# fani-lab/OpeNTF

Measured on AMD Instinct MI355X. Metric: teams/sec (train) bnn_emb d=128 on DBLP, higher is better.
Workload: dtype f32 (fp16x3 split products, f32 accumulate)

## Files before the change

opentf_amd/csrc/ntf_fused_dw.hip:

```cpp
#include "ntf_fused_common.h"

namespace ntf {

struct DwArgs {
    int B, M, Bpad;
    const float *__restrict__ dzT, *__restrict__ h, *__restrict__ hs, *__restrict__ mu, *__restrict__ rho;
    const float* wp;
    const uint32_t* sbits; int nCB; uint32_t so_k0, so_k1; int so_inj;
    float *__restrict__ g_mu, *__restrict__ g_rho, *__restrict__ g_b, *__restrict__ g_bp;
    float klw;
    float *__restrict__ w_mu, *__restrict__ w_rho, *__restrict__ m_mu, *__restrict__ v_mu, *__restrict__ m_rho, *__restrict__ v_rho;
    float lr_over_bc1, b1, b2, eps, bc2_sqrt;
    int wg_begin;
    int* rflag; int rmode;
    const uint32_t* sT;
    const uint32_t* sinT;
    const uint16_t* hb;
    float a_scale, unscale;
    int ksplit; float* part; int64_t slab; int part_row0;
    unsigned long long* stamps;
    int ntile, stagger;
    NormalSpec cur_eps; int lean;
    int produce; NormalSpec nx_eps; float* nx_wp; uint16_t *nx_pl_wp, *nx_pl_mu; float nx_pscale; double nx_klw; double* nx_kl; int* nx_rflag;
};

__device__ __forceinline__ float adam_update(float p, float g, float& m, float& v, float lr_over_bc1, float b1, float b2, float eps, float bc2_sqrt) {
    adam_step(p, g, m, v, lr_over_bc1, b1, b2, eps, __builtin_amdgcn_rcpf(bc2_sqrt));
    return p;
}

__device__ __forceinline__ uint32_t transpose32(uint32_t a, int il) {
    uint32_t m = 0x0000FFFFu;
#pragma unroll
    for (int j = 16; j != 0; j >>= 1) {
        const uint32_t pv = (uint32_t)__shfl_xor((int)a, j, 64);
        const bool lower = (il & j) == 0;
        const uint32_t lo = lower ? a : pv, hi = lower ? pv : a;
        const uint32_t t = ((lo >> j) ^ hi) & m;
        a ^= lower ? (t << j) : t;
        m ^= m << (j >> 1);
    }
    return a;
}

__device__ __forceinline__ void dw_produce_next(const DwArgs& p, int64_t idx0, const float (&mu4)[4], const float (&rho4)[4], float& kl, float& amax) {
    float z[4], ov[4];
#if defined(DWQ_ABL) && (DWQ_ABL & 2)
    z[0] = z[1] = z[2] = z[3] = 1.f;
#else
    normal4(p.nx_eps, idx0 >> 2, idx0, INT64_MAX, z);
#endif
#pragma unroll
    for (int j = 0; j < 4; ++j) {
        float ls;
        const float sigma = softplus_rho_fast(rho4[j], ls);
        ov[j] = sigma * z[j];
        kl += -ls + 0.5f * (sigma * sigma + mu4[j] * mu4[j]) - 0.5f;
    }
    if (!p.lean) *reinterpret_cast<float4*>(p.nx_wp + idx0) = make_float4(ov[0], ov[1], ov[2], ov[3]);
    const int64_t row = idx0 >> 7; const int j = (int)(idx0 & 127);
    amax = fmaxf(amax, fmaxf(fmaxf(fabsf(ov[0]), fabsf(ov[1])), fmaxf(fabsf(ov[2]), fabsf(ov[3]))));
    amax = fmaxf(amax, fmaxf(fmaxf(fabsf(mu4[0]), fabsf(mu4[1])), fmaxf(fabsf(mu4[2]), fabsf(mu4[3]))));
    planes_store_quad(p.nx_pl_wp, row, j, 128, ov[0], ov[1], ov[2], ov[3], p.nx_pscale);
    planes_store_quad(p.nx_pl_mu, row, j, 128, mu4[0], mu4[1], mu4[2], mu4[3], p.nx_pscale);
}
__device__ __forceinline__ void dw_produce_next_fnn(const DwArgs& p, int64_t idx0, const float (&mu4)[4], float& amax) {
    const int64_t row = idx0 >> 7; const int j = (int)(idx0 & 127);
    amax = fmaxf(amax, fmaxf(fmaxf(fabsf(mu4[0]), fabsf(mu4[1])), fmaxf(fabsf(mu4[2]), fabsf(mu4[3]))));
    planes_store_quad(p.nx_pl_mu, row, j, 128, mu4[0], mu4[1], mu4[2], mu4[3], p.nx_pscale);
}
template <bool BAYES = true>
__device__ __forceinline__ void dw_produce_finish(const DwArgs& p, float kl, float amax, double* red, int nwaves) {
    if (!(amax * p.nx_pscale <= 65504.f)) *p.nx_rflag = 1;
    if (!BAYES) return;
    const double s = wave_reduce_sum_d((double)kl);
    __syncthreads();
    if ((threadIdx.x & 63) == 0) red[threadIdx.x >> 6] = s;
    __syncthreads();
    if (threadIdx.x == 0) { double t = 0.0; for (int w = 0; w < nwaves; ++w) t += red[w]; atomicAdd(p.nx_kl, t * p.nx_klw); }
}

template <int H, bool BAYES, bool ADAM, int HG = H>
__device__ __forceinline__ void out_dw_f32_body(const DwArgs& p, char* smem, int jh = 0) {
    constexpr int NJT = H / 32;
    constexpr int KB = 32;
    constexpr int HROW = 4 * H;
    constexpr int TA = DW_TC * KB * 4;
    constexpr int TH = KB * HROW;
    constexpr int STAGE = TA + (BAYES ? 2 : 1) * TH;
    const int tid = threadIdx.x, lane = tid & 63, wave = tid >> 6, il = lane & 31, half = lane >> 5;
    if (range_guard_skip(p.rflag, p.rmode, false)) return;
    const int c0 = (p.wg_begin + blockIdx.x) * DW_TC;
    const int crow = wave * 32 + il;
    const int c = c0 + crow;
    const int nib = p.Bpad / KB;

    f32x16 acc1[NJT], acc2[NJT];
#pragma unroll
    for (int j = 0; j < NJT; ++j)
#pragma unroll
        for (int r = 0; r < 16; ++r) { acc1[j][r] = 0.f; acc2[j][r] = 0.f; }
    float sum1 = 0.f, sum2 = 0.f;

    const uint32_t smem_base = lds_addr(smem);
    const int wave_u = __builtin_amdgcn_readfirstlane(wave);
    auto stage = [&](int ib, int buf) {
        const uint32_t sb = smem_base + buf * STAGE;
#pragma unroll
        for (int n = 0; n < TA / 1024 / DW_WAVES; ++n) {
            const int inst = wave_u * (TA / 1024 / DW_WAVES) + n;
            const int row = inst * 8 + (lane >> 3), pch = lane & 7;
            const int q = pch ^ ((row >> 1) & 7);
            glds16(p.dzT + ((int64_t)(c0 >> 8) * nib + ib) * 8192 + row * 32 + 4 * q, sb + inst * 1024);
        }
        constexpr int HI = TH / 1024;
#pragma unroll
        for (int n = 0; n < (HI + DW_WAVES - 1) / DW_WAVES; ++n) {
            const int inst = wave_u * ((HI + DW_WAVES - 1) / DW_WAVES) + n;
            if (inst < HI) {
                int64_t goff = (int64_t)ib * KB * H + inst * 256 + lane * 4;
                if constexpr (HG != H) { const int f = inst * 256 + lane * 4; goff = (int64_t)(ib * KB + f / H) * HG + jh * H + f % H; }
                glds16(p.h + goff, sb + TA + inst * 1024);
                if (BAYES) glds16(p.hs + goff, sb + TA + TH + inst * 1024);
            }
        }
    };

    const uint32_t cb = (uint32_t)((c0 + wave * 32) >> 5);
    auto sign_col_word = [&](int ib) -> uint32_t {
        const int i = ib * KB + il;
        uint32_t w = 0u;
        if (p.so_inj) { if ((int)cb < p.nCB) w = p.sbits[(int64_t)i * p.nCB + cb]; }
        else w = sign_word(p.so_k0, p.so_k1, (uint32_t)i, cb);
        return transpose32(w, il);
    };
    uint32_t word_next = 0;
    if (BAYES) word_next = sign_col_word(0);
    stage(0, 0);
    asm volatile("s_waitcnt vmcnt(0)" ::: "memory");
    __syncthreads();
    for (int ib = 0; ib < nib; ++ib) {
        const int buf = ib & 1;
        const uint32_t word = word_next >> (4 * half);
        if (BAYES && ib + 1 < nib) word_next = sign_col_word(ib + 1);
        if (ib + 1 < nib) stage(ib + 1, buf ^ 1);
        const char* sA = smem + buf * STAGE;
        const char* sH = sA + TA;
#pragma unroll
        for (int t = 0; t < 4; ++t) {
            const int q = 2 * t + half;
            const float4 a = *reinterpret_cast<const float4*>(sA + crow * 128 + 16 * (q ^ ((crow >> 1) & 7)));
            const float av[4] = {a.x, a.y, a.z, a.w};
#pragma unroll
            for (int e4 = 0; e4 < 4; ++e4) {
                const int kk = 8 * t + e4;
                const float a1 = av[e4];
                sum1 += a1;
                float a2 = a1;
                if (BAYES) { a2 = __uint_as_float(__float_as_uint(a1) ^ ((word << (31 - kk)) & 0x80000000u)); sum2 += a2; }
                const char* hb = sH + (kk + 4 * half) * HROW + 4 * NJT * il;
                float bv[NJT], bsv[NJT];
                if (NJT == 4) {
                    const float4 b4 = *reinterpret_cast<const float4*>(hb); bv[0] = b4.x; bv[1] = b4.y; bv[NJT > 2 ? 2 : 0] = b4.z; bv[NJT > 3 ? 3 : 0] = b4.w;
                    if (BAYES) { const float4 s4 = *reinterpret_cast<const float4*>(hb + TH); bsv[0] = s4.x; bsv[1] = s4.y; bsv[NJT > 2 ? 2 : 0] = s4.z; bsv[NJT > 3 ? 3 : 0] = s4.w; }
                } else if (NJT == 2) {
                    const float2 b2 = *reinterpret_cast<const float2*>(hb); bv[0] = b2.x; bv[NJT > 1 ? 1 : 0] = b2.y;
                    if (BAYES) { const float2 s2 = *reinterpret_cast<const float2*>(hb + TH); bsv[0] = s2.x; bsv[NJT > 1 ? 1 : 0] = s2.y; }
                } else {
                    bv[0] = *reinterpret_cast<const float*>(hb);
                    if (BAYES) bsv[0] = *reinterpret_cast<const float*>(hb + TH);
                }
#pragma unroll
                for (int jt = 0; jt < NJT; ++jt) {
                    acc1[jt] = __builtin_amdgcn_mfma_f32_32x32x2f32(a1, bv[jt], acc1[jt], 0, 0, 0);
// ... 214 lines not shown
        else if (ADAM) ld_vec<NJT>(p.w_mu + idx0, v_mu);
        float a_m1[NJT], a_v1[NJT], a_m2[NJT], a_v2[NJT];
        if (ADAM) { ld_vec<NJT>(p.m_mu + idx0, a_m1); ld_vec<NJT>(p.v_mu + idx0, a_v1); if (BAYES) { ld_vec<NJT>(p.m_rho + idx0, a_m2); ld_vec<NJT>(p.v_rho + idx0, a_v2); } }
#pragma unroll
        for (int jt = 0; jt < NJT; ++jt) {
            float gm = acc1[jt][r] * p.unscale, gr = 0.f, pm = 0.f, rh = 0.f;
            if (BAYES) {
                rh = v_rho[jt];
                pm = v_mu[jt];
                const float w = v_wp[jt];
                const RhoTerms t = rho_terms_fast<true>(rh);
                gm += p.klw * pm;
                const float s2 = acc2[jt][r] * p.unscale;
                gr = (t.lo ? s2 * w : s2 * (w * t.isig) * t.sg) + p.klw * t.kl_a * t.kl_b;
            } else if (ADAM) pm = v_mu[jt];
            o_mu[jt] = gm; o_rho[jt] = gr;
            if (ADAM) {
                o_mu[jt] = adam_update(pm, gm, a_m1[jt], a_v1[jt], p.lr_over_bc1, p.b1, p.b2, p.eps, p.bc2_sqrt);
                if (BAYES) o_rho[jt] = adam_update(rh, gr, a_m2[jt], a_v2[jt], p.lr_over_bc1, p.b1, p.b2, p.eps, p.bc2_sqrt);
            }
        }
        if (!ADAM) { st_vec<NJT>(p.g_mu + idx0, o_mu); if (BAYES) st_vec<NJT>(p.g_rho + idx0, o_rho); }
        else {
            st_vec<NJT>(p.w_mu + idx0, o_mu); st_vec<NJT>(p.m_mu + idx0, a_m1); st_vec<NJT>(p.v_mu + idx0, a_v1);
            if (BAYES) { st_vec<NJT>(p.w_rho + idx0, o_rho); st_vec<NJT>(p.m_rho + idx0, a_m2); st_vec<NJT>(p.v_rho + idx0, a_v2); }
        }
    }
}


constexpr int SWT_IB = 16;
__global__ __launch_bounds__(256) void k_sign_words_T(const uint32_t* __restrict__ sbits, int so_inj, uint32_t k0, uint32_t k1, int B, int nCB, int ncb_all, int nib,
                                                      uint32_t* __restrict__ sT) {
    const int lane = threadIdx.x & 63, il = lane & 31, half = lane >> 5;
    const int cb = (blockIdx.x * 4 + (threadIdx.x >> 6)) * 2 + half;
    if (cb >= ncb_all) return;
    const int c = cb * 32 + il;
    uint32_t* dst = sT + (int64_t)(c >> 8) * nib * 256 + (c & 255);
    const int ib_end = min(nib, (int)(blockIdx.y + 1) * SWT_IB);
    for (int ib = blockIdx.y * SWT_IB; ib < ib_end; ++ib) {
        const int i = ib * 32 + il;
        uint32_t w = 0u;
        if (i < B) {
            if (so_inj) { if (cb < nCB) w = sbits[(int64_t)i * nCB + cb]; }
            else w = sign_word(k0, k1, (uint32_t)i, (uint32_t)cb);
        }
        dst[(int64_t)ib * 256] = transpose32(w, il);
    }
}

template <int N> struct DwOps { float rho[N], mu[N], m1[N], v1[N], m2[N], v2[N]; };
template <bool BAYES, bool ADAM, int N>
__device__ __forceinline__ void dw_ops_load(const DwArgs& p, int64_t idx0, DwOps<N>& o) {
    if (BAYES) { ld_vec<N>((ADAM ? p.w_rho : p.rho) + idx0, o.rho); ld_vec<N>((ADAM ? p.w_mu : p.mu) + idx0, o.mu); }
    else if (ADAM) ld_vec<N>(p.w_mu + idx0, o.mu);
    if (ADAM) { ld_vec<N>(p.m_mu + idx0, o.m1); ld_vec<N>(p.v_mu + idx0, o.v1); if (BAYES) { ld_vec<N>(p.m_rho + idx0, o.m2); ld_vec<N>(p.v_rho + idx0, o.v2); } }
}
template <bool BAYES, bool ADAM, int N>
__device__ __forceinline__ void dw_finish_ops(const DwArgs& p, int64_t idx0, const float (&s1)[N], const float (&s2)[N], DwOps<N>& o, float& nx_kl, float& nx_amax) {
    static_assert(N == 4, "one Philox quad per call");
    float o_mu[N], o_rho[N], z[4] = {0.f, 0.f, 0.f, 0.f};
#if defined(DWQ_ABL) && (DWQ_ABL & 1)
    z[0] = z[1] = z[2] = z[3] = 1.f;
#else
    if (BAYES) normal4(p.cur_eps, idx0 >> 2, idx0, INT64_MAX, z);
#endif
#pragma unroll
    for (int jt = 0; jt < N; ++jt) {
        float gm = s1[jt], gr = 0.f, pm = 0.f, rh = 0.f;
        if (BAYES) {
            rh = o.rho[jt];
            pm = o.mu[jt];
            const RhoTerms t = rho_terms_fast<true>(rh);
            gm += p.klw * pm;
            gr = s2[jt] * z[jt] * t.sg + p.klw * t.kl_a * t.kl_b;
        } else if (ADAM) pm = o.mu[jt];
        o_mu[jt] = gm; o_rho[jt] = gr;
        if (ADAM) {
            o_mu[jt] = adam_update(pm, gm, o.m1[jt], o.v1[jt], p.lr_over_bc1, p.b1, p.b2, p.eps, p.bc2_sqrt);
            if (BAYES) o_rho[jt] = adam_update(rh, gr, o.m2[jt], o.v2[jt], p.lr_over_bc1, p.b1, p.b2, p.eps, p.bc2_sqrt);
        }
    }
    if (!ADAM) { st_vec<N>(p.g_mu + idx0, o_mu); if (BAYES) st_vec<N>(p.g_rho + idx0, o_rho); }
    else {
        st_vec<N>(p.w_mu + idx0, o_mu); st_vec<N>(p.m_mu + idx0, o.m1); st_vec<N>(p.v_mu + idx0, o.v1);
        if (BAYES) { st_vec<N>(p.w_rho + idx0, o_rho); st_vec<N>(p.m_rho + idx0, o.m2); st_vec<N>(p.v_rho + idx0, o.v2); }
        if constexpr (N == 4) { if (p.produce) { if constexpr (BAYES) dw_produce_next(p, idx0, o_mu, o_rho, nx_kl, nx_amax); else dw_produce_next_fnn(p, idx0, o_mu, nx_amax); } }
    }
}
template <bool BAYES, bool ADAM, int N>
__device__ __forceinline__ void dw_finish_vec(const DwArgs& p, int64_t idx0, const float (&s1)[N], const float (&s2)[N], float& nx_kl, float& nx_amax) {
    DwOps<N> o;
    dw_ops_load<BAYES, ADAM, N>(p, idx0, o);
    dw_finish_ops<BAYES, ADAM, N>(p, idx0, s1, s2, o, nx_kl, nx_amax);
}

template <bool BAYES, bool ADAM>
__global__ __launch_bounds__(256) void k_out_dw_finish(DwArgs p) {
    if (p.rflag && *p.rflag) return;
    const int64_t q = (int64_t)blockIdx.x * 256 + threadIdx.x, il0 = q * 4, idx0 = il0 + (int64_t)p.part_row0 * 128;
    const int64_t Mp = p.slab / 128;
    if (q < Mp && q + p.part_row0 < p.M) {
        const float* pb = p.part + (int64_t)p.ksplit * 2 * p.slab;
        float b1 = 0.f, b2 = 0.f;
        for (int s = 0; s < p.ksplit; ++s) { b1 += pb[(int64_t)(s * 2) * Mp + q]; if (BAYES) b2 += pb[(int64_t)(s * 2 + 1) * Mp + q]; }
        p.g_b[q + p.part_row0] = b1; if (BAYES) p.g_bp[q + p.part_row0] = b2;
    }
    float nx_kl = 0.f, nx_amax = 0.f;
    const bool produce = ADAM && p.produce;
    const bool live = il0 < p.slab && idx0 < (int64_t)p.M * 128;
    if (!live && !produce) return;
    float s1[4] = {0.f, 0.f, 0.f, 0.f}, s2[4] = {0.f, 0.f, 0.f, 0.f};
    if (live) {
    for (int s = 0; s < p.ksplit; ++s) {
        float t[4];
        ld_vec<4>(p.part + (int64_t)(s * 2) * p.slab + il0, t);
#pragma unroll
        for (int k = 0; k < 4; ++k) s1[k] += t[k];
        if (BAYES) {
            ld_vec<4>(p.part + (int64_t)(s * 2 + 1) * p.slab + il0, t);
#pragma unroll
            for (int k = 0; k < 4; ++k) s2[k] += t[k];
        }
    }
    dw_finish_vec<BAYES, ADAM, 4>(p, idx0, s1, s2, nx_kl, nx_amax);
    }
    if (produce) { __shared__ double red[4]; dw_produce_finish<BAYES>(p, nx_kl, nx_amax, red, 4); }
}

__host__ __device__ __forceinline__ int sin_word_bit(int r) { const int g = r >> 3, q = (r & 7) >> 1, o = r & 1; return 16 * o + 4 * g + 3 - q; }
__global__ void k_sin_words_T(const uint32_t* __restrict__ sinbits, int Bpad, uint32_t* __restrict__ sinT) {
    const int t = blockIdx.x * blockDim.x + threadIdx.x;
    if (t >= (Bpad >> 5) * 128) return;
    const int ib = t >> 7, j = t & 127;
    uint32_t w = 0u;
    for (int r = 0; r < 32; ++r) w |= ((sinbits[(int64_t)(ib * 32 + r) * 4 + (j >> 5)] >> (j & 31)) & 1u) << sin_word_bit(r);
    sinT[t] = w;
}

#ifndef DW_EPI_PD
#define DW_EPI_PD 1
#endif
#ifndef DWQ_PRIO
#define DWQ_PRIO 2
#endif
#ifndef DWQ_BRING
#define DWQ_BRING 2
#endif
#ifndef DWQ_PPG
#define DWQ_PPG 3
#endif
constexpr int QW = 4;
constexpr int QTC = 32 * QW;
template <bool BAYES, bool ADAM, bool STAMP = false, bool SPLIT = false>
__global__ __launch_bounds__(64 * QW, 2) void k_out_dw_q(DwArgs p) {
    extern __shared__ __attribute__((aligned(16))) char smem[];
    constexpr int H = 128, NJT = 4;
    constexpr int TA = QTC * 32 * 4;
    constexpr int PLANE = H * 64;
    constexpr int TB = 2 * PLANE;
    constexpr int SRC_TB = (BAYES ? 2 : 1) * TB;
    constexpr int TW = BAYES ? 1024 : 0;
    constexpr int STAGE = TA + TB + TW;
    typedef _Float16 h2_t __attribute__((ext_vector_type(2)));
    const int tid = threadIdx.x, lane = tid & 63, wave = tid >> 6, il = lane & 31, half = lane >> 5;
    if (p.rmode == 1 && __builtin_nontemporal_load(p.rflag) != 0) return;
    const int ntile_s = SPLIT ? (int)gridDim.x / p.ksplit : 0;
    const int ksi = SPLIT ? (int)blockIdx.x / ntile_s : 0;
    const int c0 = (p.wg_begin + (SPLIT ? (int)blockIdx.x % ntile_s : (int)blockIdx.x)) * QTC;
    const int crow = wave * 32 + il, c = c0 + crow;
    const int nib = p.Bpad / 32;
    const int ib0 = SPLIT ? (int)((int64_t)ksi * nib / p.ksplit) : 0, ib1 = SPLIT ? (int)((int64_t)(ksi + 1) * nib / p.ksplit) : nib;
    const uint32_t smem_base = lds_addr(smem);
    const int wave_u = __builtin_amdgcn_readfirstlane(wave);
    const char* hb = reinterpret_cast<const char*>(p.hb);
    unsigned long long st_t[4] = {0, 0, 0, 0};
    if (STAMP) st_t[0] = __builtin_amdgcn_s_memrealtime();
    uint32_t lds_base = 0u;
    if (STAMP || (p.stagger > 0 && (int)blockIdx.x < p.ntile)) asm volatile("s_getreg_b32 %0, hwreg(HW_REG_LDS_ALLOC, 0, 8)" : "=s"(lds_base));
    if (p.stagger > 0 && (int)blockIdx.x < p.ntile) {
        if (lds_base != 0u) {
            const uint64_t t0 = __builtin_amdgcn_s_memrealtime();
            while (__builtin_amdgcn_s_memrealtime() - t0 < (uint64_t)p.stagger) __builtin_amdgcn_s_sleep(64);
        }
    }

    const h2_t ones = {(_Float16)1.0f, (_Float16)1.0f};
    constexpr int NA = TA / 1024 / QW, NB = TB / 1024 / QW;
    const float* dz_tile = p.dzT + (int64_t)(c0 >> 8) * nib * 8192 + ((c0 & 255) << 5);
    const uint32_t* sw_src = BAYES ? (half == 0 ? p.sT + (int64_t)(c0 >> 8) * nib * 256 + (c0 & 255) + il * 4 : p.sinT + il * 4) : nullptr;
    const int sw_step = half == 0 ? 256 : 128;
    auto stage_piece = [&](int ib, int buf, int n) {
        const uint32_t sb = smem_base + buf * STAGE;
        if (n < NA) {
            const int inst = wave_u * NA + n;
            const int row = inst * 8 + (lane >> 3), pch = lane & 7;
            const int q = pch ^ ((row >> 1) & 7);
            glds16(dz_tile + (int64_t)ib * 8192 + row * 32 + 4 * q, sb + inst * 1024);
        } else {
            const char* src = hb + (size_t)ib * SRC_TB;
            const int inst = wave_u * NB + (n - NA);
            const int pos = inst * 1024 + lane * 16;
            const int j = (pos % PLANE) >> 6, cd = (pos >> 4) & 3;
            glds16(src + (pos & ~63) + 16 * (cd ^ ((j >> 2) & 3)), sb + TA + inst * 1024);
            if (BAYES && n == NA + NB - 1) glds16(sw_src + (int64_t)ib * sw_step, sb + TA + TB);
        }
    };
    float nx_kl = 0.f, nx_amax = 0.f;
    unsigned long long st_c[3] = {0, 0, 0}, c_prev = 0;
    auto cyc = [&]() -> unsigned long long {
        unsigned long long t;
        __builtin_amdgcn_sched_barrier(0);
        asm volatile("s_memtime %0\n\ts_waitcnt lgkmcnt(0)" : "=s"(t) :: "memory");
        __builtin_amdgcn_sched_barrier(0);
        return t;
    };
#pragma unroll
    for (int n = 0; n < NA + NB; ++n) stage_piece(ib0, 0, n);
    f32x16 acc1[NJT], acc2[NJT];
#pragma unroll
    for (int j = 0; j < NJT; ++j)
#pragma unroll
        for (int r = 0; r < 16; ++r) { acc1[j][r] = 0.f; acc2[j][r] = 0.f; }
    float sum1 = 0.f, sum2 = 0.f;
    const int shl0 = 12 - 4 * half, shl1 = 4 - 4 * half;
    asm volatile("s_waitcnt vmcnt(0)" ::: "memory");
    __syncthreads();
    auto k_block = [&](int ib, auto more_c) {
        constexpr bool MORE = decltype(more_c)::value;
        const int buf = (ib - ib0) & 1;
        const char* sA = smem + buf * STAGE;
        const char* sB = sA + TA;
        uint32_t word = 0u;
        u32x4 iw = {0u, 0u, 0u, 0u};
        if (BAYES) { word = *reinterpret_cast<const uint32_t*>(sA + TA + TB + crow * 4); iw = *reinterpret_cast<const u32x4*>(sA + TA + TB + 512 + il * 16); }
        constexpr int NG = 2 * NJT;
        const char* bbase = sB + il * 64;
        const int swz = (il >> 2) & 3;
        auto load_b = [&](int g, u32x4 (&dst)[2]) {
            const int ks = g / NJT, jt = g % NJT;
            const char* bp = bbase + jt * 2048 + 16 * ((2 * ks + half) ^ swz);
#pragma unroll
            for (int q = 0; q < 2; ++q) dst[q] = *reinterpret_cast<const u32x4*>(bp + q * PLANE);
        };
        u32x4 a[2][2], as[2][2];
        auto prep_a = [&](int ks) {
            const int ch = 4 * ks + 2 * half, sw = (crow >> 1) & 7;
            const u32x4 lo = *reinterpret_cast<const u32x4*>(sA + crow * 128 + 16 * (ch ^ sw));
            const u32x4 hi = *reinterpret_cast<const u32x4*>(sA + crow * 128 + 16 * ((ch + 1) ^ sw));
            const uint32_t x[8] = {lo[0], lo[1], lo[2], lo[3], hi[0], hi[1], hi[2], hi[3]};
            const uint32_t w8 = word >> (ks * 16 + half * 8);
#pragma unroll
            for (int q = 0; q < 4; ++q) {
                const uint32_t p1 = __builtin_amdgcn_perm(x[2 * q + 1], x[2 * q], 0x05040100u), p2 = __builtin_amdgcn_perm(x[2 * q + 1], x[2 * q], 0x07060302u);
                a[ks][0][q] = p1; a[ks][1][q] = p2;
                sum1 = __builtin_amdgcn_fdot2(__builtin_bit_cast(h2_t, p1), ones, sum1, false);
                sum1 = __builtin_amdgcn_fdot2(__builtin_bit_cast(h2_t, p2), ones, sum1, false);
                if (BAYES) {
                    const uint32_t m = ((w8 << (15 - 2 * q)) & 0x8000u) | ((w8 << (30 - 2 * q)) & 0x80000000u);
                    const uint32_t s1 = p1 ^ m, s2 = p2 ^ m;
                    as[ks][0][q] = s1; as[ks][1][q] = s2;
                    sum2 = __builtin_amdgcn_fdot2(__builtin_bit_cast(h2_t, s1), ones, sum2, false);
                    sum2 = __builtin_amdgcn_fdot2(__builtin_bit_cast(h2_t, s2), ones, sum2, false);
                }
            }
        };
        constexpr int BR = DWQ_BRING;
        u32x4 bq[BR][2], bs[2];
#pragma unroll
        for (int g = 0; g < BR - 1; ++g) load_b(g, bq[g]);
        prep_a(0);
        int piece = 0;
        auto dma = [&]() {
            if (MORE) {
#pragma unroll
                for (int q = 0; q < DWQ_PPG; ++q) { if (piece < NA + NB) stage_piece(ib + 1, buf ^ 1, piece); ++piece; }
            }
        };
#pragma unroll
        for (int g = 0; g < NG; ++g) {
            if (g + BR - 1 < NG) load_b(g + BR - 1, bq[(g + BR - 1) % BR]);
            asm volatile("" ::: "memory");
            const int ks = g / NJT, jt = g % NJT;
            acc1[jt] = mfma3h(a[ks], bq[g % BR], acc1[jt]);
            dma();
            if (BAYES) {
                const uint32_t v = iw[jt] << (ks ? shl1 : shl0);
#pragma unroll
                for (int q = 0; q < 4; ++q) {
                    const uint32_t m = (v << q) & 0x80008000u;
                    bs[0][q] = bq[g % BR][0][q] ^ m; bs[1][q] = bq[g % BR][1][q] ^ m;
                }
                acc2[jt] = mfma3h(as[ks], bs, acc2[jt]);
                dma();
            }
            if (g == 0) prep_a(1);
        }
        if (STAMP) { st_c[0] += cyc() - c_prev; c_prev = cyc(); }
        asm volatile("s_waitcnt vmcnt(0)" ::: "memory");
        if (STAMP) { st_c[1] += cyc() - c_prev; c_prev = cyc(); }
        __syncthreads();
        if (STAMP) { st_c[2] += cyc() - c_prev; c_prev = cyc(); }
    };
    if (STAMP) { st_t[1] = __builtin_amdgcn_s_memrealtime(); c_prev = cyc(); }
    if (DWQ_PRIO) __builtin_amdgcn_s_setprio(DWQ_PRIO);
    for (int ib = ib0; ib < ib1 - 1; ++ib) k_block(ib, std::true_type{});
    k_block(ib1 - 1, std::false_type{});
    if (DWQ_PRIO) __builtin_amdgcn_s_setprio(0);
    if (STAMP) st_t[2] = __builtin_amdgcn_s_memrealtime();
    sum1 += __shfl_xor(sum1, 32, 64);
    sum2 += __shfl_xor(sum2, 32, 64);
    const float inv_a = 1.f / p.a_scale;
    if constexpr (SPLIT) {
        if (half == 0 && c < p.M) {
            float* pb = p.part + (int64_t)p.ksplit * 2 * p.slab; const int64_t Mp = p.slab / 128; const int cl = c - p.part_row0;
            pb[(int64_t)(ksi * 2) * Mp + cl] = sum1 * inv_a; if (BAYES) pb[(int64_t)(ksi * 2 + 1) * Mp + cl] = sum2 * inv_a;
        }
#pragma unroll
        for (int r = 0; r < 16; ++r) {
            const int cr = c0 + wave * 32 + rowmap(r, half);
            if (cr >= p.M) continue;
            const int64_t il0 = (int64_t)(cr - p.part_row0) * H + NJT * il;
            float s1[NJT], s2[NJT];
#pragma unroll
            for (int jt = 0; jt < NJT; ++jt) { s1[jt] = acc1[jt][r] * p.unscale; s2[jt] = acc2[jt][r] * p.unscale; }
            st_vec<NJT>(p.part + (int64_t)(ksi * 2) * p.slab + il0, s1);
            if (BAYES) st_vec<NJT>(p.part + (int64_t)(ksi * 2 + 1) * p.slab + il0, s2);
        }
        return;
    }
    if (half == 0 && c < p.M) { p.g_b[c] = sum1 * inv_a; if (BAYES) p.g_bp[c] = sum2 * inv_a; }

    constexpr int PD = DW_EPI_PD;
    DwOps<NJT> ops[PD + 1];
    auto row_idx = [&](int r, int64_t& idx0) -> bool {
        const int cr = c0 + wave * 32 + rowmap(r, half);
        idx0 = (int64_t)cr * H + NJT * il;
        return cr < p.M;
    };
    static_for<0, PD>([&](auto rc) { constexpr int r = decltype(rc)::value; int64_t idx0; if (row_idx(r, idx0)) dw_ops_load<BAYES, ADAM, NJT>(p, idx0, ops[r % (PD + 1)]); });
    static_for<0, 16>([&](auto rc) {
        constexpr int r = decltype(rc)::value;
        if constexpr (r + PD < 16) { int64_t idn; if (row_idx(r + PD, idn)) dw_ops_load<BAYES, ADAM, NJT>(p, idn, ops[(r + PD) % (PD + 1)]); }
        int64_t idx0;
        if (row_idx(r, idx0)) {
            float s1[NJT], s2[NJT];
#pragma unroll
            for (int jt = 0; jt < NJT; ++jt) { s1[jt] = acc1[jt][r] * p.unscale; s2[jt] = acc2[jt][r] * p.unscale; }
            dw_finish_ops<BAYES, ADAM, NJT>(p, idx0, s1, s2, ops[r % (PD + 1)], nx_kl, nx_amax);
        }
    });
    if (STAMP && p.stamps && lane == 0) {
        asm volatile("s_waitcnt vmcnt(0)" ::: "memory");
        st_t[3] = __builtin_amdgcn_s_memrealtime();
        uint32_t hw_id, xcc;
        asm volatile("s_getreg_b32 %0, hwreg(HW_REG_HW_ID)" : "=s"(hw_id));
        asm volatile("s_getreg_b32 %0, hwreg(HW_REG_XCC_ID)" : "=s"(xcc));
        unsigned long long* o = p.stamps + ((int64_t)blockIdx.x * QW + wave) * 10;
        o[0] = st_t[0]; o[1] = st_t[1]; o[2] = st_t[2]; o[3] = st_t[3]; o[4] = ((unsigned long long)xcc << 32) | hw_id; o[5] = lds_base;
        o[6] = st_c[0]; o[7] = st_c[1]; o[8] = st_c[2]; o[9] = 0;
    }
    if (ADAM && p.produce) dw_produce_finish<BAYES>(p, nx_kl, nx_amax, reinterpret_cast<double*>(smem + 2 * STAGE), QW);
}

void launch_fused_out_dw(hipStream_t st, const FusedDw& f) {
    const Geom g = geom(f.B, f.M);
    const WsLayout w = ws_layout(f.B, f.H, f.M);
    char* ws = static_cast<char*>(f.ws);
    DwArgs a;
    a.B = f.B; a.M = f.M; a.Bpad = g.Bpad; a.dzT = f.dzT; a.h = reinterpret_cast<const float*>(ws + w.hz); a.hs = reinterpret_cast<const float*>(ws + w.hs);
    a.mu = f.mu; a.rho = f.rho; a.wp = f.wp; a.sbits = reinterpret_cast<const uint32_t*>(ws + w.sbits); a.nCB = g.nCB;
    a.so_k0 = f.s_out.k0; a.so_k1 = f.s_out.k1; a.so_inj = f.s_out_inj;
    a.g_mu = f.g_mu; a.g_rho = f.g_rho; a.g_b = f.g_b; a.g_bp = f.g_bp; a.klw = f.klw;
    a.w_mu = f.w_mu; a.w_rho = f.w_rho; a.m_mu = f.m_mu; a.v_mu = f.v_mu; a.m_rho = f.m_rho; a.v_rho = f.v_rho;
    a.lr_over_bc1 = f.lr_over_bc1; a.b1 = f.b1; a.b2 = f.b2; a.eps = f.eps; a.bc2_sqrt = f.bc2_sqrt;
    const int total = (f.M + DW_TC - 1) / DW_TC;
    const int grid = f.wg_count > 0 ? std::min(f.wg_count, total - f.wg_begin) : total;
    a.wg_begin = f.wg_count > 0 ? f.wg_begin : 0;
    if (grid <= 0) return;
    a.hb = reinterpret_cast<const uint16_t*>(ws + w.hb);
    a.rflag = f.rflag; a.rmode = 0;
    a.produce = (f.produce && f.adam && f.H == 128) ? 1 : 0;
    a.cur_eps = f.cur_eps; a.lean = (a.produce && f.lean) ? 1 : 0;
    a.nx_eps = f.nx_eps; a.nx_wp = f.nx_wp; a.nx_pl_wp = f.nx_pl_wp; a.nx_pl_mu = f.nx_pl_mu; a.nx_pscale = f.nx_pscale; a.nx_klw = f.nx_klw; a.nx_kl = f.nx_kl; a.nx_rflag = f.nx_rflag;
    a.ntile = 0; a.stagger = 0; a.stamps = nullptr;
    const bool guard = f.split && f.rflag != nullptr;
    a.sT = reinterpret_cast<const uint32_t*>(ws + w.sbitsT);
    a.ksplit = 1; a.part = nullptr; a.slab = 0; a.part_row0 = 0;
    if (f.H == 256) {
        const size_t lds = 2 * ((size_t)DW_TC * 32 * 4 + (size_t)(f.bayes ? 2 : 1) * 32 * 4 * 128);
#define NTF_DWH(BY, AD) do { auto kf = k_out_dw_h2<BY, AD>; set_max_lds(reinterpret_cast<const void*>(kf), (int)lds);              \
        hipLaunchKernelGGL(kf, dim3(grid, 2), dim3(64 * DW_WAVES), lds, st, a); } while (0)
        if (f.bayes) { if (f.adam) NTF_DWH(true, true); else NTF_DWH(true, false); } else { if (f.adam) NTF_DWH(false, true); else NTF_DWH(false, false); }
#undef NTF_DWH
        return;
    }
    if (f.split && f.dz_packed) {
        a.a_scale = f.a_scale; a.unscale = 1.f / (f.a_scale * f.h_scale); a.rmode = guard ? 1 : 0;
        const int ks = (f.ksplit > 1 && f.part) ? std::min(f.ksplit, std::max(1, g.Bpad / 32)) : 1;
        if (ks > 1) {
            a.sinT = reinterpret_cast<const uint32_t*>(ws + w.sinT);
            const int total_q = (f.M + QTC - 1) / QTC, qb = f.wg_count > 0 ? 2 * f.wg_begin : 0;
            const int qgrid = f.wg_count > 0 ? std::min(2 * f.wg_count, total_q - qb) : total_q;
            const int wg256 = a.wg_begin;
            a.wg_begin = qb;
            a.ksplit = ks; a.part = f.part; a.slab = (int64_t)qgrid * QTC * 128; a.part_row0 = qb * QTC;
            const size_t ldsq = 2 * ((size_t)QTC * 128 + 2 * 128 * 64 + (f.bayes ? 1024 : 0)) + 64;
            const int64_t nq = (int64_t)qgrid * QTC * 128 / 4;
#define NTF_DWQS(BY, AD) do { auto kf = k_out_dw_q<BY, false, false, true>;                                                    \
            set_max_lds(reinterpret_cast<const void*>(kf), (int)ldsq);     \
            hipLaunchKernelGGL(kf, dim3(qgrid * ks), dim3(64 * QW), ldsq, st, a);                                              \
            hipLaunchKernelGGL((k_out_dw_finish<BY, AD>), dim3((unsigned)((nq + 255) / 256)), dim3(256), 0, st, a); } while (0)
            if (f.bayes) { if (f.adam) NTF_DWQS(true, true); else NTF_DWQS(true, false); } else { if (f.adam) NTF_DWQS(false, true); else NTF_DWQS(false, false); }
#undef NTF_DWQS
            if (!guard) return;
            a.rmode = 2; a.ksplit = 1; a.wg_begin = wg256; a.part_row0 = 0;
            goto exact_f32;
        }
        {
            a.sinT = reinterpret_cast<const uint32_t*>(ws + w.sinT);
            const int total_q = (f.M + QTC - 1) / QTC, qb = f.wg_count > 0 ? 2 * f.wg_begin : 0;
            const int qgrid = f.wg_count > 0 ? std::min(2 * f.wg_count, total_q - qb) : total_q;
            const int wg256 = a.wg_begin;
            a.wg_begin = qb;
            static int n_cu = 0;
            if (!n_cu) { int dev = 0; hipGetDevice(&dev); hipDeviceGetAttribute(&n_cu, hipDeviceAttributeMultiprocessorCount, dev); if (n_cu <= 0) n_cu = 256; }
            static const int stagger_q = getenv("NTF_DW_STAGGER") ? atoi(getenv("NTF_DW_STAGGER")) : -1;
            const int nib = g.Bpad / 32;
            a.ntile = 2 * n_cu;
            a.stagger = (f.adam && qgrid > n_cu) ? (stagger_q >= 0 ? stagger_q : (nib * 140 + 4500) / 2) : 0;
            const size_t ldsq = 2 * ((size_t)QTC * 128 + 2 * 128 * 64 + (f.bayes ? 1024 : 0)) + 64;
#define NTF_DWQ(BY, AD) do { auto kf = k_out_dw_q<BY, AD>;                                                                     \
            set_max_lds(reinterpret_cast<const void*>(kf), (int)ldsq);     \
            hipLaunchKernelGGL(kf, dim3(qgrid), dim3(64 * QW), ldsq, st, a); } while (0)
#ifdef NTF_DIAG
            static const char* stamp_file = getenv("NTF_DW_STAMP_FILE");
#else
            static const char* stamp_file = nullptr;
#endif
            if (stamp_file && f.bayes && f.adam) {
                static unsigned long long* d_st = nullptr; static int n_launch = 0;
                if (!d_st) hipMalloc(&d_st, (size_t)qgrid * QW * 10 * 8);
                a.stamps = d_st;
                auto kf = k_out_dw_q<true, true, true>;
                set_max_lds(reinterpret_cast<const void*>(kf), (int)ldsq);
                hipLaunchKernelGGL(kf, dim3(qgrid), dim3(64 * QW), ldsq, st, a);
                if (++n_launch == 30) {
                    std::vector<unsigned long long> hst((size_t)qgrid * QW * 10);
                    hipStreamSynchronize(st); hipMemcpy(hst.data(), d_st, hst.size() * 8, hipMemcpyDeviceToHost);
                    if (FILE* fp = fopen(stamp_file, "wb")) { fwrite(hst.data(), 8, hst.size(), fp); fclose(fp); }
                }
            }
            else if (f.bayes) { if (f.adam) NTF_DWQ(true, true); else NTF_DWQ(true, false); } else { if (f.adam) NTF_DWQ(false, true); else NTF_DWQ(false, false); }
#undef NTF_DWQ
            if (!guard) return;
            a.rmode = 2; a.wg_begin = wg256; a.ntile = 0; a.stagger = 0;
            goto exact_f32;
        }
    }
    if (f.split) {
        a.rmode = guard ? 1 : 0;
        a.a_scale = f.a_scale; a.unscale = 1.f / (f.a_scale * f.h_scale);
#define NTF_DWB1(HH, BY, AD) do { auto kf = k_out_dw_b6<HH, BY, AD>; const size_t lds = 2 * ((size_t)DW_TC * 128 + (size_t)(BY ? 2 : 1) * 2 * HH * 64); \
        set_max_lds(reinterpret_cast<const void*>(kf), (int)lds);                                      \
        hipLaunchKernelGGL(kf, dim3(grid), dim3(64 * DW_WAVES), lds, st, a); } while (0)
#define NTF_DWB(HH) do { if (f.bayes) { if (f.adam) NTF_DWB1(HH, true, true); else NTF_DWB1(HH, true, false); }                                            \
                         else { if (f.adam) NTF_DWB1(HH, false, true); else NTF_DWB1(HH, false, false); } } while (0)
        if (f.H == 128) NTF_DWB(128); else if (f.H == 64) NTF_DWB(64); else NTF_DWB(32);
#undef NTF_DWB
#undef NTF_DWB1
        if (!guard) return;
        a.rmode = 2;
    }
exact_f32:
    a.ntile = grid;
#define NTF_DW1(HH, BY) do { const bool fb = a.rmode == 2;                                                                                    \
        auto kf = fb ? (f.adam ? k_out_dw_fallback<HH, BY, true> : k_out_dw_fallback<HH, BY, false>) : (f.adam ? k_out_dw<HH, BY, true> : k_out_dw<HH, BY, false>);   \
        const size_t lds = 2 * (DW_TC * 32 * 4 + (BY ? 2 : 1) * 32 * 4 * HH);                                                                \
        set_max_lds(reinterpret_cast<const void*>(kf), (int)lds);                      \
        hipLaunchKernelGGL(kf, dim3(fb ? std::min(grid, 256) : grid), dim3(64 * DW_WAVES), lds, st, a); } while (0)
#define NTF_DW(HH) do { if (f.bayes) NTF_DW1(HH, true); else NTF_DW1(HH, false); } while (0)
    if (f.H == 128) NTF_DW(128); else if (f.H == 64) NTF_DW(64); else NTF_DW(32);
#undef NTF_DW
}

void launch_fused_prep_planes(hipStream_t st, int B, int H, int M, int bayes, void* ws_, float h_scale, const SignSpec* s_out, int s_out_inj, int which) {
    const Geom g = geom(B, M);
    const WsLayout w = ws_layout(B, H, M);
    char* ws = static_cast<char*>(ws_);
    if (bayes && s_out && (which & 1)) {
        const int ncb_all = rup(M, DW_TC) / 32, nib = g.Bpad / 32;
        hipLaunchKernelGGL(k_sign_words_T, dim3((ncb_all + 7) / 8, (nib + SWT_IB - 1) / SWT_IB), dim3(256), 0, st, reinterpret_cast<const uint32_t*>(ws + w.sbits), s_out_inj, s_out->k0, s_out->k1,
                           B, g.nCB, ncb_all, nib, reinterpret_cast<uint32_t*>(ws + w.sbitsT));
    }
    if (!(which & 2)) return;
    const int n = g.Bpad * H;
    hipLaunchKernelGGL(k_prep_planes_T, dim3((n + 255) / 256), dim3(256), 0, st, reinterpret_cast<const float*>(ws + w.hz), reinterpret_cast<const float*>(ws + w.hs),
                       bayes, g.Bpad, H, h_scale, reinterpret_cast<uint16_t*>(ws + w.hb));
    if (bayes && H == 128)
        hipLaunchKernelGGL(k_sin_words_T, dim3((g.Bpad / 32 * 128 + 255) / 256), dim3(256), 0, st, reinterpret_cast<const uint32_t*>(ws + w.sinbits), g.Bpad, reinterpret_cast<uint32_t*>(ws + w.sinT));
}

}
```

profiles/dw_stamps.py:

```python
import numpy as np, sys
a = np.fromfile(sys.argv[1], dtype=np.uint64).reshape(-1, 4, 10)
w0 = a[:, 0, :]
t0 = w0[:, 0].min()
ent = (w0[:, 0] - t0) / 100.0; mb = (w0[:, 1] - t0) / 100.0; me = (w0[:, 2] - t0) / 100.0; ex = (w0[:, 3] - t0) / 100.0
hw = w0[:, 4] & 0xffffffff; xcc = w0[:, 4] >> 32; lds = w0[:, 5]
cu = ((xcc.astype(np.int64) & 15) << 8) | ((hw.astype(np.int64) >> 8) & 0xff)
print("workgroups", len(w0), "distinct CUs", len(np.unique(cu)), "kernel span us", ex.max())
print("lds_base values", np.unique(lds, return_counts=True))
print("first-round (first 512) lds_base != 0:", int((lds[:512] != 0).sum()))
print("main loop us: mean %.1f  p10 %.1f p90 %.1f | epilogue us: mean %.1f p10 %.1f p90 %.1f | stagger wait mean %.1f" % (
    (me - mb).mean(), np.percentile(me - mb, 10), np.percentile(me - mb, 90), (ex - me).mean(), np.percentile(ex - me, 10), np.percentile(ex - me, 90), (mb - ent).mean()))
tot_ov = 0.0; tot_main2 = 0.0; tot_epi2 = 0.0; tot = 0.0
for c in np.unique(cu):
    idx = np.where(cu == c)[0]
    ev = []
    for i in idx: ev += [(mb[i], 'm', 1), (me[i], 'm', -1), (me[i], 'e', 1), (ex[i], 'e', -1)]
    ev.sort()
    nm = ne = 0; last = ev[0][0]
    for t, k, d in ev:
        dt = t - last; last = t
        if nm >= 1 and ne >= 1: tot_ov += dt
        if nm >= 2: tot_main2 += dt
        if ne >= 2: tot_epi2 += dt
        tot += dt
        if k == 'm': nm += d
        else: ne += d
print("cycles per K block and wave (all waves): body %.0f | DMA wait %.0f | barrier %.0f" % tuple(a[:, :, 6 + k].mean() / 32 for k in range(3)))
print("per-CU time: main||epilogue %.1f %%  two main loops %.1f %%  two epilogues %.1f %%" % (100 * tot_ov / tot, 100 * tot_main2 / tot, 100 * tot_epi2 / tot))
c = np.unique(cu)[3]
idx = np.where(cu == c)[0]; idx = idx[np.argsort(ent[idx])]
print("CU", hex(c))
for i in idx: print("  wg %5d lds %3d enter %7.1f main %7.1f..%7.1f exit %7.1f" % (i, lds[i], ent[i], mb[i], me[i], ex[i]))
```

Before: 673,700.

## Shrink dW workgroup tile to 64 experts with hidden-split waves for 3 WGs/CU

```diff
diff --git a/opentf_amd/csrc/ntf_fused_dw.hip b/opentf_amd/csrc/ntf_fused_dw.hip
--- a/opentf_amd/csrc/ntf_fused_dw.hip
+++ b/opentf_amd/csrc/ntf_fused_dw.hip
@@ -20,6 +20,7 @@
     int ksplit; float* part; int64_t slab; int part_row0;
     unsigned long long* stamps;
     int ntile, stagger;
+    int lds_third;
     NormalSpec cur_eps; int lean;
     int produce; NormalSpec nx_eps; float* nx_wp; uint16_t *nx_pl_wp, *nx_pl_mu; float nx_pscale; double nx_klw; double* nx_kl; int* nx_rflag;
 };
@@ -540,10 +541,14 @@
 #endif
 constexpr int QW = 4;
 constexpr int QTC = 32 * QW;
-template <bool BAYES, bool ADAM, bool STAMP = false, bool SPLIT = false>
-__global__ __launch_bounds__(64 * QW, 2) void k_out_dw_q(DwArgs p) {
+constexpr int QTC_U = 64;
+template <bool BAYES, bool ADAM, bool STAMP = false, bool SPLIT = false, bool U64 = false>
+__global__ __launch_bounds__(64 * QW, U64 ? 3 : 2) void k_out_dw_q(DwArgs p) {
     extern __shared__ __attribute__((aligned(16))) char smem[];
+    static_assert(!(U64 && SPLIT), "the split-K launches use the 128-expert form");
     constexpr int H = 128, NJT = 4;
+    constexpr int NT = U64 ? 2 : 4;
+    constexpr int QTC = U64 ? QTC_U : ntf::QTC;
     constexpr int TA = QTC * 32 * 4;
     constexpr int PLANE = H * 64;
     constexpr int TB = 2 * PLANE;
@@ -556,7 +561,8 @@
     const int ntile_s = SPLIT ? (int)gridDim.x / p.ksplit : 0;
     const int ksi = SPLIT ? (int)blockIdx.x / ntile_s : 0;
     const int c0 = (p.wg_begin + (SPLIT ? (int)blockIdx.x % ntile_s : (int)blockIdx.x)) * QTC;
-    const int crow = wave * 32 + il, c = c0 + crow;
+    const int ew = U64 ? (wave & 1) : wave, hw = U64 ? (wave >> 1) : 0;
+    const int crow = ew * 32 + il, c = c0 + crow;
     const int nib = p.Bpad / 32;
     const int ib0 = SPLIT ? (int)((int64_t)ksi * nib / p.ksplit) : 0, ib1 = SPLIT ? (int)((int64_t)(ksi + 1) * nib / p.ksplit) : nib;
     const uint32_t smem_base = lds_addr(smem);
@@ -565,18 +571,19 @@
     unsigned long long st_t[4] = {0, 0, 0, 0};
     if (STAMP) st_t[0] = __builtin_amdgcn_s_memrealtime();
     uint32_t lds_base = 0u;
-    if (STAMP || (p.stagger > 0 && (int)blockIdx.x < p.ntile)) asm volatile("s_getreg_b32 %0, hwreg(HW_REG_LDS_ALLOC, 0, 8)" : "=s"(lds_base));
+    if (STAMP || (p.stagger > 0 && (int)blockIdx.x < p.ntile)) asm volatile("s_getreg_b32 %0, hwreg(HW_REG_LDS_ALLOC, 0, 12)" : "=s"(lds_base));
     if (p.stagger > 0 && (int)blockIdx.x < p.ntile) {
         if (lds_base != 0u) {
+            const uint64_t wait = (uint64_t)p.stagger * ((U64 && (int)lds_base >= p.lds_third) ? 2u : 1u);
             const uint64_t t0 = __builtin_amdgcn_s_memrealtime();
-            while (__builtin_amdgcn_s_memrealtime() - t0 < (uint64_t)p.stagger) __builtin_amdgcn_s_sleep(64);
+            while (__builtin_amdgcn_s_memrealtime() - t0 < wait) __builtin_amdgcn_s_sleep(64);
         }
     }
 
     const h2_t ones = {(_Float16)1.0f, (_Float16)1.0f};
     constexpr int NA = TA / 1024 / QW, NB = TB / 1024 / QW;
     const float* dz_tile = p.dzT + (int64_t)(c0 >> 8) * nib * 8192 + ((c0 & 255) << 5);
-    const uint32_t* sw_src = BAYES ? (half == 0 ? p.sT + (int64_t)(c0 >> 8) * nib * 256 + (c0 & 255) + il * 4 : p.sinT + il * 4) : nullptr;
+    const uint32_t* sw_src = BAYES ? (half == 0 ? p.sT + (int64_t)(c0 >> 8) * nib * 256 + (c0 & 255) + ((il * 4) & (QTC - 1)) : p.sinT + il * 4) : nullptr;
     const int sw_step = half == 0 ? 256 : 128;
     auto stage_piece = [&](int ib, int buf, int n) {
         const uint32_t sb = smem_base + buf * STAGE;
@@ -590,7 +597,9 @@
             const int inst = wave_u * NB + (n - NA);
             const int pos = inst * 1024 + lane * 16;
             const int j = (pos % PLANE) >> 6, cd = (pos >> 4) & 3;
-            glds16(src + (pos & ~63) + 16 * (cd ^ ((j >> 2) & 3)), sb + TA + inst * 1024);
+            const int u = 64 * (j >> 6) + 2 * (j & 31) + ((j >> 5) & 1);
+            const int spos = U64 ? (pos - (pos % PLANE)) + (32 * (u & 3) + (u >> 2)) * 64 : (pos & ~63);
+            glds16(src + spos + 16 * (cd ^ ((j >> 2) & 3)), sb + TA + inst * 1024);
             if (BAYES && n == NA + NB - 1) glds16(sw_src + (int64_t)ib * sw_step, sb + TA + TB);
         }
     };
@@ -605,9 +614,9 @@
     };
 #pragma unroll
     for (int n = 0; n < NA + NB; ++n) stage_piece(ib0, 0, n);
-    f32x16 acc1[NJT], acc2[NJT];
-#pragma unroll
-    for (int j = 0; j < NJT; ++j)
+    f32x16 acc1[NT], acc2[NT];
+#pragma unroll
+    for (int j = 0; j < NT; ++j)
 #pragma unroll
         for (int r = 0; r < 16; ++r) { acc1[j][r] = 0.f; acc2[j][r] = 0.f; }
     float sum1 = 0.f, sum2 = 0.f;
@@ -620,14 +629,20 @@
         const char* sA = smem + buf * STAGE;
         const char* sB = sA + TA;
         uint32_t word = 0u;
-        u32x4 iw = {0u, 0u, 0u, 0u};
-        if (BAYES) { word = *reinterpret_cast<const uint32_t*>(sA + TA + TB + crow * 4); iw = *reinterpret_cast<const u32x4*>(sA + TA + TB + 512 + il * 16); }
-        constexpr int NG = 2 * NJT;
+        uint32_t iw[NT];
+#pragma unroll
+        for (int t = 0; t < NT; ++t) iw[t] = 0u;
+        if (BAYES) {
+            word = *reinterpret_cast<const uint32_t*>(sA + TA + TB + crow * 4);
+            if constexpr (U64) { const uint2 w2 = *reinterpret_cast<const uint2*>(sA + TA + TB + 512 + (64 * hw + 2 * il) * 4); iw[0] = w2.x; iw[1] = w2.y; }
+            else { const u32x4 w4 = *reinterpret_cast<const u32x4*>(sA + TA + TB + 512 + il * 16); iw[0] = w4[0]; iw[1] = w4[1]; iw[NT > 2 ? 2 : 0] = w4[2]; iw[NT > 3 ? 3 : 0] = w4[3]; }
+        }
+        constexpr int NG = 2 * NT;
         const char* bbase = sB + il * 64;
         const int swz = (il >> 2) & 3;
         auto load_b = [&](int g, u32x4 (&dst)[2]) {
-            const int ks = g / NJT, jt = g % NJT;
-            const char* bp = bbase + jt * 2048 + 16 * ((2 * ks + half) ^ swz);
+            const int ks = g / NT, jt = g % NT;
+            const char* bp = bbase + (hw * NT + jt) * 2048 + 16 * ((2 * ks + half) ^ swz);
 #pragma unroll
             for (int q = 0; q < 2; ++q) dst[q] = *reinterpret_cast<const u32x4*>(bp + q * PLANE);
         };
@@ -669,7 +684,7 @@
         for (int g = 0; g < NG; ++g) {
             if (g + BR - 1 < NG) load_b(g + BR - 1, bq[(g + BR - 1) % BR]);
             asm volatile("" ::: "memory");
-            const int ks = g / NJT, jt = g % NJT;
+            const int ks = g / NT, jt = g % NT;
             acc1[jt] = mfma3h(a[ks], bq[g % BR], acc1[jt]);
             dma();
             if (BAYES) {
@@ -717,10 +732,37 @@
         }
         return;
     }
-    if (half == 0 && c < p.M) { p.g_b[c] = sum1 * inv_a; if (BAYES) p.g_bp[c] = sum2 * inv_a; }
+    if (half == 0 && c < p.M && hw == 0) { p.g_b[c] = sum1 * inv_a; if (BAYES) p.g_bp[c] = sum2 * inv_a; }
 
     constexpr int PD = DW_EPI_PD;
     DwOps<NJT> ops[PD + 1];
+    if constexpr (U64) {
+        const bool odd = (il & 1) != 0;
+        auto row_idx = [&](int k, int64_t& idx0) -> bool {
+            const int cr = c0 + ew * 32 + rowmap(2 * k + (odd ? 1 : 0), half);
+            idx0 = (int64_t)cr * H + 64 * hw + 4 * (il >> 1);
+            return cr < p.M;
+        };
+        static_for<0, PD>([&](auto kc) { constexpr int k = decltype(kc)::value; int64_t idx0; if (row_idx(k, idx0)) dw_ops_load<BAYES, ADAM, NJT>(p, idx0, ops[k % (PD + 1)]); });
+        static_for<0, 8>([&](auto kc) {
+            constexpr int k = decltype(kc)::value;
+            if constexpr (k + PD < 8) { int64_t idn; if (row_idx(k + PD, idn)) dw_ops_load<BAYES, ADAM, NJT>(p, idn, ops[(k + PD) % (PD + 1)]); }
+            float s1[NJT], s2[NJT];
+#pragma unroll
+            for (int t = 0; t < 2; ++t) {
+                const float own1 = odd ? acc1[t][2 * k + 1] : acc1[t][2 * k], give1 = odd ? acc1[t][2 * k] : acc1[t][2 * k + 1];
+                const float got1 = __shfl_xor(give1, 1, 64);
+                s1[t] = (odd ? got1 : own1) * p.unscale; s1[2 + t] = (odd ? own1 : got1) * p.unscale;
+                if (BAYES) {
+                    const float own2 = odd ? acc2[t][2 * k + 1] : acc2[t][2 * k], give2 = odd ? acc2[t][2 * k] : acc2[t][2 * k + 1];
+                    const float got2 = __shfl_xor(give2, 1, 64);
+                    s2[t] = (odd ? got2 : own2) * p.unscale; s2[2 + t] = (odd ? own2 : got2) * p.unscale;
+                } else { s2[t] = 0.f; s2[2 + t] = 0.f; }
+            }
+            int64_t idx0;
+            if (row_idx(k, idx0)) dw_finish_ops<BAYES, ADAM, NJT>(p, idx0, s1, s2, ops[k % (PD + 1)], nx_kl, nx_amax);
+        });
+    } else {
     auto row_idx = [&](int r, int64_t& idx0) -> bool {
         const int cr = c0 + wave * 32 + rowmap(r, half);
         idx0 = (int64_t)cr * H + NJT * il;
@@ -738,6 +780,7 @@
             dw_finish_ops<BAYES, ADAM, NJT>(p, idx0, s1, s2, ops[r % (PD + 1)], nx_kl, nx_amax);
         }
     });
+    }
     if (STAMP && p.stamps && lane == 0) {
         asm volatile("s_waitcnt vmcnt(0)" ::: "memory");
         st_t[3] = __builtin_amdgcn_s_memrealtime();
@@ -771,7 +814,7 @@
     a.produce = (f.produce && f.adam && f.H == 128) ? 1 : 0;
     a.cur_eps = f.cur_eps; a.lean = (a.produce && f.lean) ? 1 : 0;
     a.nx_eps = f.nx_eps; a.nx_wp = f.nx_wp; a.nx_pl_wp = f.nx_pl_wp; a.nx_pl_mu = f.nx_pl_mu; a.nx_pscale = f.nx_pscale; a.nx_klw = f.nx_klw; a.nx_kl = f.nx_kl; a.nx_rflag = f.nx_rflag;
-    a.ntile = 0; a.stagger = 0; a.stamps = nullptr;
+    a.ntile = 0; a.stagger = 0; a.lds_third = 0; a.stamps = nullptr;
     const bool guard = f.split && f.rflag != nullptr;
     a.sT = reinterpret_cast<const uint32_t*>(ws + w.sbitsT);
     a.ksplit = 1; a.part = nullptr; a.slab = 0; a.part_row0 = 0;
@@ -807,18 +850,20 @@
         }
         {
             a.sinT = reinterpret_cast<const uint32_t*>(ws + w.sinT);
-            const int total_q = (f.M + QTC - 1) / QTC, qb = f.wg_count > 0 ? 2 * f.wg_begin : 0;
-            const int qgrid = f.wg_count > 0 ? std::min(2 * f.wg_count, total_q - qb) : total_q;
+            constexpr int per256 = DW_TC / QTC_U;
+            const int total_q = (f.M + QTC_U - 1) / QTC_U, qb = f.wg_count > 0 ? per256 * f.wg_begin : 0;
+            const int qgrid = f.wg_count > 0 ? std::min(per256 * f.wg_count, total_q - qb) : total_q;
             const int wg256 = a.wg_begin;
             a.wg_begin = qb;
             static int n_cu = 0;
             if (!n_cu) { int dev = 0; hipGetDevice(&dev); hipDeviceGetAttribute(&n_cu, hipDeviceAttributeMultiprocessorCount, dev); if (n_cu <= 0) n_cu = 256; }
             static const int stagger_q = getenv("NTF_DW_STAGGER") ? atoi(getenv("NTF_DW_STAGGER")) : -1;
             const int nib = g.Bpad / 32;
-            a.ntile = 2 * n_cu;
-            a.stagger = (f.adam && qgrid > n_cu) ? (stagger_q >= 0 ? stagger_q : (nib * 140 + 4500) / 2) : 0;
-            const size_t ldsq = 2 * ((size_t)QTC * 128 + 2 * 128 * 64 + (f.bayes ? 1024 : 0)) + 64;
-#define NTF_DWQ(BY, AD) do { auto kf = k_out_dw_q<BY, AD>;                                                                     \
+            const size_t ldsq = 2 * ((size_t)QTC_U * 128 + 2 * 128 * 64 + (f.bayes ? 1024 : 0)) + 64;
+            a.ntile = 3 * n_cu;
+            a.stagger = (f.adam && qgrid > n_cu) ? (stagger_q >= 0 ? stagger_q : (nib * 100 + 3000) / 3) : 0;
+            a.lds_third = (int)(ldsq * 3 / 2 / 256);
+#define NTF_DWQ(BY, AD) do { auto kf = k_out_dw_q<BY, AD, false, false, true>;                                                                     \
             set_max_lds(reinterpret_cast<const void*>(kf), (int)ldsq);     \
             hipLaunchKernelGGL(kf, dim3(qgrid), dim3(64 * QW), ldsq, st, a); } while (0)
 #ifdef NTF_DIAG
@@ -830,7 +875,7 @@
                 static unsigned long long* d_st = nullptr; static int n_launch = 0;
                 if (!d_st) hipMalloc(&d_st, (size_t)qgrid * QW * 10 * 8);
                 a.stamps = d_st;
-                auto kf = k_out_dw_q<true, true, true>;
+                auto kf = k_out_dw_q<true, true, true, false, true>;
                 set_max_lds(reinterpret_cast<const void*>(kf), (int)ldsq);
                 hipLaunchKernelGGL(kf, dim3(qgrid), dim3(64 * QW), ldsq, st, a);
                 if (++n_launch == 30) {
diff --git a/profiles/dw_stamps.py b/profiles/dw_stamps.py
--- a/profiles/dw_stamps.py
+++ b/profiles/dw_stamps.py
@@ -1,5 +1,6 @@
 import numpy as np, sys
-a = np.fromfile(sys.argv[1], dtype=np.uint64).reshape(-1, 4, 10)
+qw = int(sys.argv[2]) if len(sys.argv) > 2 else 4
+a = np.fromfile(sys.argv[1], dtype=np.uint64).reshape(-1, qw, 10)
 w0 = a[:, 0, :]
 t0 = w0[:, 0].min()
 ent = (w0[:, 0] - t0) / 100.0; mb = (w0[:, 1] - t0) / 100.0; me = (w0[:, 2] - t0) / 100.0; ex = (w0[:, 3] - t0) / 100.0
@@ -11,22 +12,27 @@
 print("main loop us: mean %.1f  p10 %.1f p90 %.1f | epilogue us: mean %.1f p10 %.1f p90 %.1f | stagger wait mean %.1f" % (
     (me - mb).mean(), np.percentile(me - mb, 10), np.percentile(me - mb, 90), (ex - me).mean(), np.percentile(ex - me, 10), np.percentile(ex - me, 90), (mb - ent).mean()))
 tot_ov = 0.0; tot_main2 = 0.0; tot_epi2 = 0.0; tot = 0.0
+busy = {}; span = ex.max()
 for c in np.unique(cu):
     idx = np.where(cu == c)[0]
     ev = []
     for i in idx: ev += [(mb[i], 'm', 1), (me[i], 'm', -1), (me[i], 'e', 1), (ex[i], 'e', -1)]
     ev.sort()
     nm = ne = 0; last = ev[0][0]
+    busy[0] = busy.get(0, 0.0) + ev[0][0] + (span - ev[-1][0])
     for t, k, d in ev:
         dt = t - last; last = t
         if nm >= 1 and ne >= 1: tot_ov += dt
         if nm >= 2: tot_main2 += dt
         if ne >= 2: tot_epi2 += dt
+        busy[nm + ne] = busy.get(nm + ne, 0.0) + dt
         tot += dt
         if k == 'm': nm += d
         else: ne += d
 print("cycles per K block and wave (all waves): body %.0f | DMA wait %.0f | barrier %.0f" % tuple(a[:, :, 6 + k].mean() / 32 for k in range(3)))
 print("per-CU time: main||epilogue %.1f %%  two main loops %.1f %%  two epilogues %.1f %%" % (100 * tot_ov / tot, 100 * tot_main2 / tot, 100 * tot_epi2 / tot))
+nb = sum(busy.values())
+print("per-CU time over the launch (%.1f us): " % span + "  ".join("%s %.1f %%" % ({0: "none", 1: "one workgroup alone"}.get(k, "%d at work" % k), 100 * v / nb) for k, v in sorted(busy.items())))
 c = np.unique(cu)[3]
 idx = np.where(cu == c)[0]; idx = idx[np.argsort(ent[idx])]
 print("CU", hex(c))
```

After: 640,000. 5.0% lower.
